# SerezD/gen_adversarial

Hardware: AMD Instinct MI355X
Metric: purified images/sec (attack+encode+decode) (higher is better)
Workload: dtype f32 storage; contractions as 3x bf16 MFMA (hi/lo split), fp32 accumulate; 1 GPU; configs[1]: NVAE purify + VGG-11, 64x64, PGD-Linf step (fwd + input-grad), bs 256 images/GPU x EoT 32 = 8192 defender rows per step, alphas ours_cosine_no_preprocessing_ids.yaml x0.7, assumed NVAE config (C=32, 3x8 groups, 20 latents); images_per_gpu=256, eot=32, rows_per_gpu=8192, chunk_rows=1024, streams=2, parallelism=image-sharded x1

## Files before the change

### gen_adversarial_amd/csrc/dwconv5.hip

```cpp
#include "ga_common.h"

namespace ga {

constexpr int DW_CC = 32;

template <int SW>
__global__ void __launch_bounds__(256, 4)
dwconv5_kernel(const ga_dwconv5_desc d, const int NB, const int TH, const int TW, const int tilesH, const int tilesW,
               const int nchunks) {
    extern __shared__ __attribute__((aligned(16))) float smem[];
    const int tid = threadIdx.x, c4 = tid & 7, pl = tid >> 3;

    int b = blockIdx.x;
    const int chunk = b % nchunks; b /= nchunks;
    const int tw = b % tilesW; b /= tilesW;
    const int th = b % tilesH; b /= tilesH;
    const int n0 = b * NB;
    const int nb = min(NB, d.N - n0);
    const int h0 = th * TH, w0 = tw * TW;
    const int c = chunk * DW_CC + 4 * c4;
    const bool cok = c < d.C;

    const int HH = TH + 4, WW = TW + 4;
    const int Hs = d.up2 ? d.H / 2 : d.H, Ws = d.up2 ? d.W / 2 : d.W;
    float* wS = smem;
    float* tile = smem + 25 * DW_CC;

    const floatx4 zero = {0.f, 0.f, 0.f, 0.f};
    if (tid < 200) {
        const int t = tid >> 3;
        *reinterpret_cast<floatx4*>(wS + t * DW_CC + 4 * c4) =
            cok ? *reinterpret_cast<const floatx4*>(d.w + (size_t)t * d.C + c) : zero;
    }
    floatx4 bias = zero;
    if (cok && d.bias) bias = *reinterpret_cast<const floatx4*>(d.bias + c);

    const int halo_px = nb * HH * WW;
    for (int p0 = pl; p0 < halo_px; p0 += 32 * 4) {
        floatx4 v[4];
        bool ok[4];
#pragma unroll
        for (int k = 0; k < 4; ++k) {
            const int p = p0 + 32 * k;
            const int ww = p % WW; const int q = p / WW;
            const int hh = q % HH; const int ni = q / HH;
            const int h = h0 + hh - 2, w = w0 + ww - 2;
            ok[k] = cok && p < halo_px && h >= 0 && h < d.H && w >= 0 && w < d.W;
            const int hs = d.up2 ? (h >> 1) : h, ws = d.up2 ? (w >> 1) : w;
            const size_t off = ok[k] ? (((size_t)(n0 + ni) * Hs + hs) * Ws + ws) * d.C + c : 0;
            v[k] = *reinterpret_cast<const floatx4*>(d.x + off);
        }
#pragma unroll
        for (int k = 0; k < 4; ++k) {
            const int p = p0 + 32 * k;
            if (p < halo_px) {
                floatx4 o = v[k];
                if (d.pro_act == GA_ACT_SILU) {
#pragma unroll
                    for (int e = 0; e < 4; ++e) o[e] = o[e] * fast_sigmoid(o[e]);
                } else if (d.pro_act) {
#pragma unroll
                    for (int e = 0; e < 4; ++e) o[e] = act_fwd_fast(o[e], d.pro_act);
                }
                *reinterpret_cast<floatx4*>(tile + (size_t)p * DW_CC + 4 * c4) = ok[k] ? o : zero;
            }
        }
    }
    __syncthreads();
    if (!cok) return;

    auto strip = [&](const int ni, const int hh, const int ws, floatx4 (&acc)[SW]) {
#pragma unroll
        for (int j = 0; j < SW; ++j) acc[j] = zero;
        const float* base = tile + ((size_t)(ni * HH + hh) * WW + ws) * DW_CC + 4 * c4;
#pragma unroll 1
        for (int kh = 0; kh < 5; ++kh) {
            floatx4 w5[5], in[SW + 4];
#pragma unroll
            for (int kw = 0; kw < 5; ++kw) w5[kw] = *reinterpret_cast<const floatx4*>(wS + (kh * 5 + kw) * DW_CC + 4 * c4);
#pragma unroll
            for (int j = 0; j < SW + 4; ++j) in[j] = *reinterpret_cast<const floatx4*>(base + (kh * WW + j) * DW_CC);
#pragma unroll
            for (int j = 0; j < SW; ++j)
#pragma unroll
                for (int kw = 0; kw < 5; ++kw) acc[j] += in[j + kw] * w5[kw];
        }
    };

    const size_t row_out = (size_t)(d.pool2 ? (d.H / 2) * (d.W / 2) : d.H * d.W) * d.C;
    const int arep = d.act_rep > 1 ? d.act_rep : 1;
    auto finish = [&](floatx4 v, const int n, const size_t po) __attribute__((always_inline)) {
        const size_t o = (size_t)n * row_out + po;
        if (d.dact_x) {
            const floatx4 u = *reinterpret_cast<const floatx4*>(d.dact_x + (size_t)(n / arep) * row_out + po);
            if (d.dact_act == GA_ACT_SILU) {
#pragma unroll
                for (int e = 0; e < 4; ++e) { const float sg = fast_sigmoid(u[e]); v[e] *= sg * (1.0f + u[e] * (1.0f - sg)); }
            } else {
#pragma unroll
                for (int e = 0; e < 4; ++e) v[e] *= act_bwd_fast(u[e], d.dact_act);
            }
        }
        *reinterpret_cast<floatx4*>(d.y + o) = v;
    };

    const int th_n = min(TH, d.H - h0), tw_n = min(TW, d.W - w0);
    if (!d.pool2) {
        const int spr = (tw_n + SW - 1) / SW;
        const int nst = nb * th_n * spr;
        for (int s = pl; s < nst; s += 32) {
            const int sx = s % spr; const int q = s / spr;
            const int hh = q % th_n; const int ni = q / th_n;
            floatx4 acc[SW];
            strip(ni, hh, sx * SW, acc);
#pragma unroll
            for (int j = 0; j < SW; ++j) {
                const int ww = sx * SW + j;
                if (ww < tw_n)
                    finish(acc[j] + bias, n0 + ni, ((size_t)(h0 + hh) * d.W + (w0 + ww)) * d.C + c);
            }
        }
    } else {
        const int Wo = d.W / 2;
        const int spr = (tw_n + SW - 1) / SW;
        const int nst = nb * (th_n / 2) * spr;
        for (int s = pl; s < nst; s += 32) {
            const int sx = s % spr; const int q = s / spr;
            const int hr = q % (th_n / 2); const int ni = q / (th_n / 2);
            floatx4 a0[SW], a1[SW];
            strip(ni, 2 * hr, sx * SW, a0);
            strip(ni, 2 * hr + 1, sx * SW, a1);
#pragma unroll
            for (int j = 0; j < SW; j += 2) {
                const int ww = sx * SW + j;
                if (ww < tw_n) {
                    const floatx4 v = a0[j] + a0[j + (SW > 1 ? 1 : 0)] + a1[j] + a1[j + (SW > 1 ? 1 : 0)];
                    finish(v + bias, n0 + ni, ((size_t)(h0 / 2 + hr) * Wo + (w0 + ww) / 2) * d.C + c);
                }
            }
        }
    }
}

__global__ void __launch_bounds__(256, 4) dwconv5_4x4_kernel(const ga_dwconv5_desc d, const int nchunks) {
    constexpr int NB = 16;
    __shared__ __attribute__((aligned(16))) float wS[25 * DW_CC];
    __shared__ __attribute__((aligned(16))) float tile[NB * 16 * DW_CC];
    const int tid = threadIdx.x, c4 = tid & 7, pl = tid >> 3;
    const int chunk = blockIdx.x % nchunks;
    const int n0 = (blockIdx.x / nchunks) * NB;
    const int nb = min(NB, d.N - n0);
    const int c = chunk * DW_CC + 4 * c4;
    const bool cok = c < d.C;
    const floatx4 zero = {0.f, 0.f, 0.f, 0.f};
    if (tid < 200) {
        const int t = tid >> 3;
        *reinterpret_cast<floatx4*>(wS + t * DW_CC + 4 * c4) = cok ? *reinterpret_cast<const floatx4*>(d.w + (size_t)t * d.C + c) : zero;
    }
    floatx4 bias = zero;
    if (cok && d.bias) bias = *reinterpret_cast<const floatx4*>(d.bias + c);
    {
        floatx4 v[8];
#pragma unroll
        for (int k = 0; k < 8; ++k) {
            const int p = pl + 32 * k;
            const bool ok = cok && p < nb * 16;
            v[k] = ok ? *reinterpret_cast<const floatx4*>(d.x + ((size_t)n0 * 16 + p) * d.C + c) : zero;
        }
#pragma unroll
        for (int k = 0; k < 8; ++k) {
            const int p = pl + 32 * k;
            floatx4 o = v[k];
            if (d.pro_act == GA_ACT_SILU) {
#pragma unroll
                for (int e = 0; e < 4; ++e) o[e] = o[e] * fast_sigmoid(o[e]);
            } else if (d.pro_act) {
#pragma unroll
                for (int e = 0; e < 4; ++e) o[e] = act_fwd_fast(o[e], d.pro_act);
            }
            *reinterpret_cast<floatx4*>(tile + p * DW_CC + 4 * c4) = o;
        }
    }
    __syncthreads();
    if (!cok) return;
    for (int s = pl; s < nb * 4; s += 32) {
        const int ni = s >> 2, h = s & 3;
        floatx4 acc[4] = {bias, bias, bias, bias};
        const int kh0 = max(0, 2 - h), kh1 = min(5, 6 - h);
        for (int kh = kh0; kh < kh1; ++kh) {
            const float* row = tile + ((ni * 4 + h + kh - 2) * 4) * DW_CC + 4 * c4;
            floatx4 in[4], w5[5];
#pragma unroll
            for (int j = 0; j < 4; ++j) in[j] = *reinterpret_cast<const floatx4*>(row + j * DW_CC);
#pragma unroll
            for (int kw = 0; kw < 5; ++kw) w5[kw] = *reinterpret_cast<const floatx4*>(wS + (kh * 5 + kw) * DW_CC + 4 * c4);
#pragma unroll
            for (int w = 0; w < 4; ++w)
#pragma unroll
                for (int j = 0; j < 4; ++j) {
                    const int kw = j - w + 2;
                    if (kw >= 0 && kw < 5) acc[w] += in[j] * w5[kw];
                }
        }
#pragma unroll
        for (int w = 0; w < 4; ++w) {
            const size_t o = (((size_t)(n0 + ni) * 4 + h) * 4 + w) * d.C + c;
            floatx4 v = acc[w];
            if (d.dact_x) {
                const int na = d.act_rep > 1 ? (n0 + ni) / d.act_rep : n0 + ni;
                const floatx4 u = *reinterpret_cast<const floatx4*>(d.dact_x + (((size_t)na * 4 + h) * 4 + w) * d.C + c);
                if (d.dact_act == GA_ACT_SILU) {
#pragma unroll
                    for (int e = 0; e < 4; ++e) { const float sg = fast_sigmoid(u[e]); v[e] *= sg * (1.0f + u[e] * (1.0f - sg)); }
                } else {
#pragma unroll
                    for (int e = 0; e < 4; ++e) v[e] *= act_bwd_fast(u[e], d.dact_act);
                }
            }
            *reinterpret_cast<floatx4*>(d.y + o) = v;
        }
    }
}

}

extern "C" int ga_dwconv5(const ga_dwconv5_desc* dp, void* stream_) {
    ga::clear_stale_error();
    using namespace ga;
    if (!dp) return GA_E_BADARG;
    const ga_dwconv5_desc& d = *dp;
    if (!d.x || !d.w || !d.y || d.N <= 0 || d.H <= 0 || d.W <= 0 || d.C <= 0) return GA_E_BADARG;
    if (d.C % 4) return GA_E_UNSUPPORTED;
    if ((d.up2 || d.pool2) && ((d.H | d.W) & 1)) return GA_E_BADARG;
    if (d.up2 && d.pool2) return GA_E_UNSUPPORTED;
    if (d.act_rep > 1 && d.N % d.act_rep) return GA_E_BADARG;
    if (!aligned16(d.x) || !aligned16(d.w) || !aligned16(d.y) || (d.bias && !aligned16(d.bias)) ||
        (d.dact_x && !aligned16(d.dact_x))) return GA_E_ALIGN;
    hipStream_t stream = reinterpret_cast<hipStream_t>(stream_);

    if (d.H == 4 && d.W == 4 && !d.up2 && !d.pool2) {
        const int nchunks = (d.C + DW_CC - 1) / DW_CC;
        const long blocks = (long)((d.N + 15) / 16) * nchunks;
        if (blocks > 0x7fffffffL) return GA_E_UNSUPPORTED;
        hipLaunchKernelGGL(dwconv5_4x4_kernel, dim3((unsigned)blocks), dim3(256), 0, stream, d, nchunks);
        return check_launch();
    }
    const int TH = d.H < 8 ? d.H : 8, TW = d.W < 16 ? d.W : 16;
    const int halo_bytes = (TH + 4) * (TW + 4) * DW_CC * 4;
    int NB = 256 / (TH * TW);
    if (NB < 1) NB = 1;
    const int fit = (40 * 1024 - 25 * DW_CC * 4) / halo_bytes;
    if (NB > fit) NB = fit;
    if (NB > d.N) NB = d.N;
    if (NB < 1) NB = 1;
    const int tilesH = (d.H + TH - 1) / TH, tilesW = (d.W + TW - 1) / TW;
    const int nchunks = (d.C + DW_CC - 1) / DW_CC;
    const long blocks = (long)((d.N + NB - 1) / NB) * tilesH * tilesW * nchunks;
    if (blocks > 0x7fffffffL) return GA_E_UNSUPPORTED;
    const size_t lds = (size_t)NB * halo_bytes + 25 * DW_CC * 4;
    const bool w2 = (d.W % 2 == 0) && (TW % 2 == 0);
    const bool w4 = (d.W % 4 == 0) && (TW % 4 == 0) && !(w2 && NB * TH * (TW / 4) < 32);
    if (w4) hipLaunchKernelGGL(dwconv5_kernel<4>, dim3((unsigned)blocks), dim3(256), lds, stream, d, NB, TH, TW, tilesH, tilesW, nchunks);
    else if (w2) hipLaunchKernelGGL(dwconv5_kernel<2>, dim3((unsigned)blocks), dim3(256), lds, stream, d, NB, TH, TW, tilesH, tilesW, nchunks);
    else {
        if (d.pool2) return GA_E_UNSUPPORTED;
        hipLaunchKernelGGL(dwconv5_kernel<1>, dim3((unsigned)blocks), dim3(256), lds, stream, d, NB, TH, TW, tilesH, tilesW, nchunks);
    }
    return check_launch();
}
```

Measured before the change: 6287 defender rows/s (rows = images x EoT-32).

## Add dedicated upsample-by-2 depthwise 5x5 kernel staging low-res tiles

Adds a separate kernel for the nearest-upsample (up2) depthwise 5x5 case. It stages the low-resolution source tile in LDS instead of a replicated high-resolution halo, and splits channels into two planes of 16 floats to reduce bank conflicts. Each thread computes a 2x4 output patch by reusing shared low-res inputs. This cuts LDS footprint and global loads for the upsampled layers in the NVAE decoder. The generic kernel drops its up2 handling, and the epilogue is moved into shared device helpers.

```diff
diff --git a/gen_adversarial_amd/csrc/dwconv5.hip b/gen_adversarial_amd/csrc/dwconv5.hip
--- a/gen_adversarial_amd/csrc/dwconv5.hip
+++ b/gen_adversarial_amd/csrc/dwconv5.hip
@@ -3,6 +3,23 @@
 namespace ga {
 
 constexpr int DW_CC = 32;
+
+__device__ __forceinline__ floatx4 dw_dact(const ga_dwconv5_desc& d, floatx4 v, const floatx4 u) {
+    if (d.dact_act == GA_ACT_SILU) {
+#pragma unroll
+        for (int e = 0; e < 4; ++e) { const float sg = fast_sigmoid(u[e]); v[e] *= sg * (1.0f + u[e] * (1.0f - sg)); }
+    } else {
+#pragma unroll
+        for (int e = 0; e < 4; ++e) v[e] *= act_bwd_fast(u[e], d.dact_act);
+    }
+    return v;
+}
+
+__device__ __forceinline__ void dw_finish(const ga_dwconv5_desc& d, floatx4 v, const int n, const size_t po,
+                                          const size_t row_out, const int arep) {
+    if (d.dact_x) v = dw_dact(d, v, *reinterpret_cast<const floatx4*>(d.dact_x + (size_t)(n / arep) * row_out + po));
+    *reinterpret_cast<floatx4*>(d.y + (size_t)n * row_out + po) = v;
+}
 
 template <int SW>
 __global__ void __launch_bounds__(256, 4)
@@ -22,7 +39,6 @@
     const bool cok = c < d.C;
 
     const int HH = TH + 4, WW = TW + 4;
-    const int Hs = d.up2 ? d.H / 2 : d.H, Ws = d.up2 ? d.W / 2 : d.W;
     float* wS = smem;
     float* tile = smem + 25 * DW_CC;
 
@@ -46,8 +62,7 @@
             const int hh = q % HH; const int ni = q / HH;
             const int h = h0 + hh - 2, w = w0 + ww - 2;
             ok[k] = cok && p < halo_px && h >= 0 && h < d.H && w >= 0 && w < d.W;
-            const int hs = d.up2 ? (h >> 1) : h, ws = d.up2 ? (w >> 1) : w;
-            const size_t off = ok[k] ? (((size_t)(n0 + ni) * Hs + hs) * Ws + ws) * d.C + c : 0;
+            const size_t off = ok[k] ? (((size_t)(n0 + ni) * d.H + h) * d.W + w) * d.C + c : 0;
             v[k] = *reinterpret_cast<const floatx4*>(d.x + off);
         }
 #pragma unroll
@@ -89,21 +104,6 @@
 
     const size_t row_out = (size_t)(d.pool2 ? (d.H / 2) * (d.W / 2) : d.H * d.W) * d.C;
     const int arep = d.act_rep > 1 ? d.act_rep : 1;
-    auto finish = [&](floatx4 v, const int n, const size_t po) __attribute__((always_inline)) {
-        const size_t o = (size_t)n * row_out + po;
-        if (d.dact_x) {
-            const floatx4 u = *reinterpret_cast<const floatx4*>(d.dact_x + (size_t)(n / arep) * row_out + po);
-            if (d.dact_act == GA_ACT_SILU) {
-#pragma unroll
-                for (int e = 0; e < 4; ++e) { const float sg = fast_sigmoid(u[e]); v[e] *= sg * (1.0f + u[e] * (1.0f - sg)); }
-            } else {
-#pragma unroll
-                for (int e = 0; e < 4; ++e) v[e] *= act_bwd_fast(u[e], d.dact_act);
-            }
-        }
-        *reinterpret_cast<floatx4*>(d.y + o) = v;
-    };
-
     const int th_n = min(TH, d.H - h0), tw_n = min(TW, d.W - w0);
     if (!d.pool2) {
         const int spr = (tw_n + SW - 1) / SW;
@@ -117,7 +117,7 @@
             for (int j = 0; j < SW; ++j) {
                 const int ww = sx * SW + j;
                 if (ww < tw_n)
-                    finish(acc[j] + bias, n0 + ni, ((size_t)(h0 + hh) * d.W + (w0 + ww)) * d.C + c);
+                    dw_finish(d, acc[j] + bias, n0 + ni, ((size_t)(h0 + hh) * d.W + (w0 + ww)) * d.C + c, row_out, arep);
             }
         }
     } else {
@@ -135,10 +135,119 @@
                 const int ww = sx * SW + j;
                 if (ww < tw_n) {
                     const floatx4 v = a0[j] + a0[j + (SW > 1 ? 1 : 0)] + a1[j] + a1[j + (SW > 1 ? 1 : 0)];
-                    finish(v + bias, n0 + ni, ((size_t)(h0 / 2 + hr) * Wo + (w0 + ww) / 2) * d.C + c);
-                }
-            }
-        }
+                    dw_finish(d, v + bias, n0 + ni, ((size_t)(h0 / 2 + hr) * Wo + (w0 + ww) / 2) * d.C + c, row_out, arep);
+                }
+            }
+        }
+    }
+}
+
+
+__device__ __forceinline__ void dw_stage_split(const ga_dwconv5_desc& d, float* tq, const int n0, const int nb, const int HH,
+                                               const int WW, const int hb, const int wb, const int Hi, const int Wi,
+                                               const int c, const bool cok, const int pl) {
+    const floatx4 zero = {0.f, 0.f, 0.f, 0.f};
+    const int npx = nb * HH * WW;
+    for (int p0 = pl; p0 < npx; p0 += 32 * 8) {
+        floatx4 v[8];
+        bool ok[8];
+#pragma unroll
+        for (int k = 0; k < 8; ++k) {
+            const int p = p0 + 32 * k;
+            const int ww = p % WW; const int q = p / WW;
+            const int hh = q % HH; const int ni = q / HH;
+            const int h = hb + hh, w = wb + ww;
+            ok[k] = cok && p < npx && h >= 0 && h < Hi && w >= 0 && w < Wi;
+            const size_t off = ok[k] ? (((size_t)(n0 + ni) * Hi + h) * Wi + w) * d.C + c : 0;
+            v[k] = *reinterpret_cast<const floatx4*>(d.x + off);
+        }
+#pragma unroll
+        for (int k = 0; k < 8; ++k) {
+            const int p = p0 + 32 * k;
+            if (p < npx) {
+                floatx4 o = v[k];
+                if (d.pro_act == GA_ACT_SILU) {
+#pragma unroll
+                    for (int e = 0; e < 4; ++e) o[e] = o[e] * fast_sigmoid(o[e]);
+                } else if (d.pro_act) {
+#pragma unroll
+                    for (int e = 0; e < 4; ++e) o[e] = act_fwd_fast(o[e], d.pro_act);
+                }
+                *reinterpret_cast<floatx4*>(tq + (size_t)p * 16) = ok[k] ? o : zero;
+            }
+        }
+    }
+}
+
+__global__ void __launch_bounds__(256, 4)
+dwconv5_up2_kernel(const ga_dwconv5_desc d, const int NB, const int TH, const int TW, const int WW, const int plane,
+                   const int tilesH, const int tilesW, const int nchunks) {
+    extern __shared__ __attribute__((aligned(16))) float smem[];
+    const int tid = threadIdx.x, c4 = tid & 7, pl = tid >> 3;
+
+    int b = blockIdx.x;
+    const int chunk = b % nchunks; b /= nchunks;
+    const int tw = b % tilesW; b /= tilesW;
+    const int th = b % tilesH; b /= tilesH;
+    const int n0 = b * NB;
+    const int nb = min(NB, d.N - n0);
+    const int Hs = d.H / 2, Ws = d.W / 2;
+    const int h0 = th * TH, w0 = tw * TW;
+    const int c = chunk * DW_CC + 4 * c4;
+    const bool cok = c < d.C;
+    const int HH = TH + 2;
+    float* wS = smem;
+    float* tq = smem + 25 * DW_CC + (c4 >> 2) * plane + 4 * (c4 & 3);
+
+    const floatx4 zero = {0.f, 0.f, 0.f, 0.f};
+    if (tid < 200) {
+        const int t = tid >> 3;
+        *reinterpret_cast<floatx4*>(wS + t * DW_CC + 4 * c4) =
+            cok ? *reinterpret_cast<const floatx4*>(d.w + (size_t)t * d.C + c) : zero;
+    }
+    floatx4 bias = zero;
+    if (cok && d.bias) bias = *reinterpret_cast<const floatx4*>(d.bias + c);
+    dw_stage_split(d, tq, n0, nb, HH, WW, h0 - 1, w0 - 1, Hs, Ws, c, cok, pl);
+    __syncthreads();
+    if (!cok) return;
+
+    const size_t row_out = (size_t)d.H * d.W * d.C;
+    const int arep = d.act_rep > 1 ? d.act_rep : 1;
+    const int th_n = min(TH, Hs - h0), tw_n = min(TW, Ws - w0);
+    const int spr = (tw_n + 1) / 2;
+    const int nst = nb * th_n * spr;
+    for (int it = pl; it < nst; it += 32) {
+        const int sx = it % spr; const int q = it / spr;
+        const int i = q % th_n; const int ni = q / th_n;
+        floatx4 acc[2][4];
+#pragma unroll
+        for (int a = 0; a < 2; ++a)
+#pragma unroll
+            for (int k = 0; k < 4; ++k) acc[a][k] = zero;
+        const float* base = tq + ((size_t)(ni * HH + i) * WW + 2 * sx) * 16;
+#pragma unroll 1
+        for (int kh = 0; kh < 5; ++kh) {
+            floatx4 w5[5];
+#pragma unroll
+            for (int kw = 0; kw < 5; ++kw) w5[kw] = *reinterpret_cast<const floatx4*>(wS + (kh * 5 + kw) * DW_CC + 4 * c4);
+#pragma unroll
+            for (int a = 0; a < 2; ++a) {
+                floatx4 in[4];
+#pragma unroll
+                for (int k = 0; k < 4; ++k) in[k] = *reinterpret_cast<const floatx4*>(base + (((a + kh) >> 1) * WW + k) * 16);
+#pragma unroll
+                for (int k = 0; k < 4; ++k)
+#pragma unroll
+                    for (int kw = 0; kw < 5; ++kw) acc[a][k] += in[(k >> 1) + (((k & 1) + kw) >> 1)] * w5[kw];
+            }
+        }
+#pragma unroll
+        for (int a = 0; a < 2; ++a)
+#pragma unroll
+            for (int k = 0; k < 4; ++k)
+                if (2 * sx + (k >> 1) < tw_n)
+                    dw_finish(d, acc[a][k] + bias, n0 + ni,
+                              ((size_t)(2 * (h0 + i) + a) * d.W + (2 * (w0 + 2 * sx) + k)) * d.C + c, row_out, arep);
     }
 }
 
@@ -238,11 +347,31 @@
         (d.dact_x && !aligned16(d.dact_x))) return GA_E_ALIGN;
     hipStream_t stream = reinterpret_cast<hipStream_t>(stream_);
 
+    const int nchunks = (d.C + DW_CC - 1) / DW_CC;
     if (d.H == 4 && d.W == 4 && !d.up2 && !d.pool2) {
-        const int nchunks = (d.C + DW_CC - 1) / DW_CC;
         const long blocks = (long)((d.N + 15) / 16) * nchunks;
         if (blocks > 0x7fffffffL) return GA_E_UNSUPPORTED;
         hipLaunchKernelGGL(dwconv5_4x4_kernel, dim3((unsigned)blocks), dim3(256), 0, stream, d, nchunks);
+        return check_launch();
+    }
+    if (d.up2) {
+        const int Hs = d.H / 2, Ws = d.W / 2;
+        const int TH = Hs < 8 ? Hs : 8, TW = Ws < 16 ? Ws : 16;
+        const int HH = TH + 2, WW = ((TW + 1) & ~1) + 2;
+        const int items = TH * ((TW + 1) / 2);
+        int NB = 64 / items;
+        const int fit = (32 * 1024 - 25 * DW_CC * 4 - 2 * 80 * 4) / (HH * WW * DW_CC * 4);
+        if (NB > fit) NB = fit;
+        const int per32 = 32 / items;
+        if (per32 > 1 && NB > per32) NB -= NB % per32;
+        if (NB > d.N) NB = d.N;
+        if (NB < 1) NB = 1;
+        const int plane = ((NB * HH * WW * 16 + 63) & ~63) + 16;
+        const int tilesH = (Hs + TH - 1) / TH, tilesW = (Ws + TW - 1) / TW;
+        const long blocks = (long)((d.N + NB - 1) / NB) * tilesH * tilesW * nchunks;
+        if (blocks > 0x7fffffffL) return GA_E_UNSUPPORTED;
+        const size_t lds = (size_t)(25 * DW_CC + 2 * plane) * 4;
+        hipLaunchKernelGGL(dwconv5_up2_kernel, dim3((unsigned)blocks), dim3(256), lds, stream, d, NB, TH, TW, WW, plane, tilesH, tilesW, nchunks);
         return check_launch();
     }
     const int TH = d.H < 8 ? d.H : 8, TW = d.W < 16 ? d.W : 16;
@@ -254,7 +383,6 @@
     if (NB > d.N) NB = d.N;
     if (NB < 1) NB = 1;
     const int tilesH = (d.H + TH - 1) / TH, tilesW = (d.W + TW - 1) / TW;
-    const int nchunks = (d.C + DW_CC - 1) / DW_CC;
     const long blocks = (long)((d.N + NB - 1) / NB) * tilesH * tilesW * nchunks;
     if (blocks > 0x7fffffffL) return GA_E_UNSUPPORTED;
     const size_t lds = (size_t)NB * halo_bytes + 25 * DW_CC * 4;
```

Result: faster. 6359 defender rows/s (rows = images x EoT-32), median of 6 (+1.2%).
